# Hengle/AkariRender-1

Hardware: AMD Instinct MI355X
Metric: Msamples/sec (whole node), 10M-tri scene 1080p 1024spp, 1/2/4/8 MI355X (higher is better)
Workload: dtype f32; 1 GPU; C3 synthetic triangle soup (SURVEY.md §8d); triangles=10000002, width=1920, height=1080, spp=1025, max_depth=5, tile=64, parallelism=tile-split x1, bvh_leaf=4, builder=sbvh, form=k_path, ordered_fetch=True

## Files before the change

akarirender-1_amd/csrc/kernels.hip:

```cpp
#include "akr_device.h"
#include "akr_math.h"
#include "kernels.h"

namespace akr {

__device__ __forceinline__ uint32_t fbits(float f) { return __float_as_uint(f); }
__device__ __forceinline__ float bitsf(uint32_t u) { return __uint_as_float(u); }

template <bool TIGHT, bool FAST = false>
__device__ __forceinline__ float box_test(float lox, float hix, float loy, float hiy, float loz, float hiz, V3 o,
                                          V3 invd, float tmin, float tmax) {
    float t0x = (lox - o.x) * invd.x, t1x = (hix - o.x) * invd.x;
    float t0y = (loy - o.y) * invd.y, t1y = (hiy - o.y) * invd.y;
    float t0z = (loz - o.z) * invd.z, t1z = (hiz - o.z) * invd.z;
    float m0, m1, t;
    if (FAST) {
        m0 = fmaxf(fmaxf(fminf(t0x, t1x), fminf(t0y, t1y)), fminf(t0z, t1z));
        m1 = fminf(fminf(fmaxf(t0x, t1x), fmaxf(t0y, t1y)), fmaxf(t0z, t1z));
        t = fmaxf(tmin, m0);
    } else {
        m0 = rmax(rmax(rmin(t0x, t1x), rmin(t0y, t1y)), rmin(t0z, t1z));
        m1 = rmin(rmin(rmax(t0x, t1x), rmax(t0y, t1y)), rmax(t0z, t1z));
        t = rmax(tmin, m0);
    }
// ... 76 lines not shown
    pos_b = bb + lane_prefix(mb);
}

__device__ __forceinline__ void issue_together(const float4 &a, const float4 &b, const float4 &c, const float4 &d,
                                               const float4 &e, const float4 &f) {
    asm volatile("" ::"v"(a.x), "v"(a.y), "v"(a.z), "v"(a.w), "v"(b.x), "v"(b.y), "v"(b.z), "v"(c.x), "v"(c.y),
                 "v"(c.z), "v"(d.x), "v"(d.y), "v"(d.z), "v"(d.w), "v"(e.x), "v"(e.y), "v"(e.z), "v"(f.x), "v"(f.y),
                 "v"(f.z));
}

#define AKR_CHILD_POP 0xFFFFFFFEu
__device__ __forceinline__ bool is_internal(uint32_t c) { return !(c & AKR_CHILD_LEAF); }
__device__ __forceinline__ bool is_leaf(uint32_t c) { return (c & AKR_CHILD_LEAF) && c < AKR_CHILD_POP; }

typedef __attribute__((address_space(3))) unsigned long long lds_u64;
typedef __attribute__((address_space(1))) unsigned long long glb_u64;

constexpr int kStackLdsU64 = kStackLds * kTraceBlock;
__device__ __forceinline__ unsigned long long lds_get(const lds_u64 *s, int e, uint32_t tid) {
    return s[e * kTraceBlock + tid];
}
__device__ __forceinline__ void lds_put(lds_u64 *s, int e, uint32_t tid, unsigned long long v) {
    s[e * kTraceBlock + tid] = v;
}

__device__ __forceinline__ uint32_t stack_pop(const lds_u64 *s_stack, const glb_u64 *ovf, uint32_t ovf_threads,
                                              uint32_t tid, uint32_t gtid, int &sp, float lim) {
    if (__ballot(sp > kStackLds) == 0) {
        while (sp > 0) {
            --sp;
            const unsigned long long e = lds_get(s_stack, sp, tid);
            if (!(__uint_as_float((uint32_t)(e >> 32)) > lim)) return (uint32_t)e;
        }
        return AKR_CHILD_EMPTY;
    }
    while (sp > 0) {
        --sp;
        unsigned long long e;
        if (sp < kStackLds) e = lds_get(s_stack, sp, tid);
        else e = ovf[(size_t)(sp - kStackLds) * ovf_threads + gtid];
        if (!(__uint_as_float((uint32_t)(e >> 32)) > lim)) return (uint32_t)e;
    }
    return AKR_CHILD_EMPTY;
}

template <bool TIGHT, bool FAST, bool ANY>
__device__ __forceinline__ void visit_node(const float4 *nodesf, const uint4 *nodesu, uint32_t &cur, V3 o, V3 d,
                                           V3 invd, float tmin, float tmax, float best, lds_u64 *s_stack, glb_u64 *ovf,
                                           uint32_t ovf_threads, uint32_t tid, uint32_t gtid, int &sp) {
    const float4 q0 = nodesf[4 * (size_t)cur + 0];
    const float4 q1 = nodesf[4 * (size_t)cur + 1];
    const float4 q2 = nodesf[4 * (size_t)cur + 2];
    const uint4 q3 = nodesu[4 * (size_t)cur + 3];
    const float t0 = box_test<TIGHT, FAST>(q0.x, q0.y, q0.z, q0.w, q2.x, q2.y, o, invd, tmin, tmax);
    const float t1 = box_test<TIGHT, FAST>(q1.x, q1.y, q1.z, q1.w, q2.z, q2.w, o, invd, tmin, tmax);
    const float lim = ANY ? tmax : best;
    const bool p0 = !(t0 < 0.0f || t0 > lim);
    const bool p1 = !(t1 < 0.0f || t1 > lim);
    const float dax = q3.z == 0 ? d.x : (q3.z == 1 ? d.y : d.z);
    const bool left_first = dax > 0;
    const uint32_t near_ref = left_first ? q3.x : q3.y;
    const uint32_t far_ref = left_first ? q3.y : q3.x;
    const bool pn = left_first ? p0 : p1;
    const bool pf = left_first ? p1 : p0;
    const float tf = left_first ? t1 : t0;
    if (pn && pf) {
        const unsigned long long e = (unsigned long long)far_ref | ((unsigned long long)__float_as_uint(tf) << 32);
        if (sp < kStackLds) lds_put(s_stack, sp, tid, e);
        else ovf[(size_t)(sp - kStackLds) * ovf_threads + gtid] = e;
        sp++;
    }
    cur = pn ? near_ref : (pf ? far_ref : stack_pop(s_stack, ovf, ovf_threads, tid, gtid, sp, lim));
}

__device__ __forceinline__ float ubyte(uint32_t w, int k) {
    return (float)((w >> (8 * k)) & 0xFFu);
}

template <bool ANY, bool NOPOP = false, bool FIT = false>
__device__ __forceinline__ bool wide_order_push(uint32_t order_lo, uint32_t order_hi, uint32_t dpos, const float (&t)[4],
                                                const bool (&hit)[4], const uint32_t (&ref)[4], uint32_t &cur, float lim,
                                                lds_u64 *s_stack, glb_u64 *ovf, uint32_t ovf_threads, uint32_t tid,
                                                uint32_t gtid, int &sp, lds_u64 *dead = nullptr,
                                                uint32_t *info = nullptr) {
    const uint32_t perm = ((dpos & 4u) ? order_hi : order_lo) >> ((dpos & 3u) << 3);
    const uint32_t pos[4] = {perm & 3u, (perm >> 2) & 3u, (perm >> 4) & 3u, (perm >> 6) & 3u};
    uint32_t pm = 0;
#pragma unroll
    for (int k = 0; k < 4; k++) pm |= hit[k] ? (1u << pos[k]) : 0u;
    if (pm == 0) {
        if constexpr (NOPOP) return true;
        cur = stack_pop(s_stack, ovf, ovf_threads, tid, gtid, sp, lim);
        return false;
    }
    const uint32_t rest = pm & (pm - 1u);
    if (info)
        *info = 1u | (sp + 4 > kStackLds ? 2u : 0u) | (sp + (int)__popc(rest) > kStackLds ? 4u : 0u);
    const bool all_lds = FIT ? __ballot(sp + (int)__popc(rest) > kStackLds) == 0 : __ballot(sp + 4 > kStackLds) == 0;
    if (all_lds) {
#pragma unroll
        for (int k = 0; k < 4; k++) {
            const bool push = (rest >> pos[k]) & 1u;
            const unsigned long long v = (unsigned long long)ref[k] | ((unsigned long long)__float_as_uint(t[k]) << 32);
            if constexpr (FIT) {
                lds_u64 *p = push ? s_stack + (sp + (int)__popc(rest >> (pos[k] + 1u))) * kTraceBlock + tid : dead;
                *p = v;
            } else {
                const int e = sp + (push ? (int)__popc(rest >> (pos[k] + 1u)) : 3);
                lds_put(s_stack, e, tid, v);
            }
        }
    } else {
#pragma unroll
        for (int k = 0; k < 4; k++) {
            if ((rest >> pos[k]) & 1u) {
                const int e = sp + (int)__popc(rest >> (pos[k] + 1u));
                const unsigned long long v = (unsigned long long)ref[k] | ((unsigned long long)__float_as_uint(t[k]) << 32);
                if (e < kStackLds) lds_put(s_stack, e, tid, v);
                else ovf[(size_t)(e - kStackLds) * ovf_threads + gtid] = v;
            }
        }
    }
    sp += (int)__popc(rest);
    const uint32_t first = pm ^ rest;
    uint32_t c = AKR_CHILD_EMPTY;
#pragma unroll
    for (int k = 0; k < 4; k++) c = ((first >> pos[k]) & 1u) ? ref[k] : c;
    cur = c;
    return false;
}

template <bool TIGHT, bool ANY>
__device__ __forceinline__ int visit_wide(const float4 *wn, uint32_t &cur, V3 o, uint32_t dpos, V3 invd, float tmin, float tmax,
                                          float best, lds_u64 *s_stack, glb_u64 *ovf, uint32_t ovf_threads,
                                          uint32_t tid, uint32_t gtid, int &sp) {
    const char *wb = reinterpret_cast<const char *>(wn);
    const uint32_t off = cur << 6;
    const float4 h = *reinterpret_cast<const float4 *>(wb + off);
    const uint4 c = *reinterpret_cast<const uint4 *>(wb + off + 16);
    const uint4 qa = *reinterpret_cast<const uint4 *>(wb + off + 32);
    const uint4 qb = *reinterpret_cast<const uint4 *>(wb + off + 48);
    const uint32_t meta = __float_as_uint(h.w);
    const float sx = __uint_as_float((meta & 0xFFu) << 23);
    const float sy = __uint_as_float(((meta >> 8) & 0xFFu) << 23);
    const float sz = __uint_as_float(((meta >> 16) & 0xFFu) << 23);
    const float lim = ANY ? tmax : best;
    float t[4];
    bool hit[4];
    uint32_t ref[4] = {c.x, c.y, c.z, c.w};
#pragma unroll
    for (int k = 0; k < 4; k++) {
        const float lox = __builtin_fmaf(ubyte(qa.x, k), sx, h.x), hix = __builtin_fmaf(ubyte(qa.y, k), sx, h.x);
        const float loy = __builtin_fmaf(ubyte(qa.z, k), sy, h.y), hiy = __builtin_fmaf(ubyte(qa.w, k), sy, h.y);
        const float loz = __builtin_fmaf(ubyte(qb.x, k), sz, h.z), hiz = __builtin_fmaf(ubyte(qb.y, k), sz, h.z);
        t[k] = box_test<TIGHT, true>(lox, hix, loy, hiy, loz, hiz, o, invd, tmin, tmax);
        hit[k] = ref[k] != AKR_CHILD_EMPTY && !(t[k] < 0.0f || t[k] > lim);
    }
    const int tested = (c.x != AKR_CHILD_EMPTY) + (c.y != AKR_CHILD_EMPTY) + (c.z != AKR_CHILD_EMPTY) +
                       (c.w != AKR_CHILD_EMPTY);
    wide_order_push<ANY>(qb.z, qb.w, dpos, t, hit, ref, cur, lim, s_stack, ovf, ovf_threads, tid, gtid, sp);
    return tested;
}

struct WideNode {
    float4 h;
    uint4 c, qa, qb;
};
__device__ __forceinline__ WideNode wide_load(const float4 *wn, uint32_t cur) {
    const char *wb = reinterpret_cast<const char *>(wn);
    const uint32_t off = cur << 6;
    WideNode nd;
    nd.h = *reinterpret_cast<const float4 *>(wb + off);
    nd.c = *reinterpret_cast<const uint4 *>(wb + off + 16);
    nd.qa = *reinterpret_cast<const uint4 *>(wb + off + 32);
    nd.qb = *reinterpret_cast<const uint4 *>(wb + off + 48);
    return nd;
}

template <bool ANY, bool NOPOP = false, bool FIT = false>
__device__ __forceinline__ int visit_wide_lean_node(const WideNode &nd, uint32_t &cur, V3 o, uint32_t dpos, V3 invd,
                                                    float tmin, float tmaxp, float best, lds_u64 *s_stack, glb_u64 *ovf,
                                                    uint32_t ovf_threads, uint32_t tid, uint32_t gtid, int &sp,
                                                    bool *need_pop = nullptr, lds_u64 *dead = nullptr,
                                                    uint32_t *push_info = nullptr) {
    const float4 h = nd.h;
    const uint4 c = nd.c, qa = nd.qa, qb = nd.qb;
    const uint32_t meta = __float_as_uint(h.w);
    constexpr float kRel = 0x1p-21f;
    constexpr float kAbs = 0x1p-120f;
    const float scx = __uint_as_float((meta & 0xFFu) << 23) * invd.x;
    const float scy = __uint_as_float(((meta >> 8) & 0xFFu) << 23) * invd.y;
    const float scz = __uint_as_float(((meta >> 16) & 0xFFu) << 23) * invd.z;
    const float oqx = (h.x - o.x) * invd.x, oqy = (h.y - o.y) * invd.y, oqz = (h.z - o.z) * invd.z;
    const float ex = __builtin_fmaf(__builtin_fmaf(255.0f, fabsf(scx), fabsf(oqx)), kRel, kAbs);
    const float ey = __builtin_fmaf(__builtin_fmaf(255.0f, fabsf(scy), fabsf(oqy)), kRel, kAbs);
    const float ez = __builtin_fmaf(__builtin_fmaf(255.0f, fabsf(scz), fabsf(oqz)), kRel, kAbs);
    const float nox = oqx - ex, noy = oqy - ey, noz = oqz - ez;
    const float fox = oqx + ex, foy = oqy + ey, foz = oqz + ez;
    const bool px = invd.x > 0.0f, py = invd.y > 0.0f, pz = invd.z > 0.0f;
    const uint32_t qnx = px ? qa.x : qa.y, qfx = px ? qa.y : qa.x;
    const uint32_t qny = py ? qa.z : qa.w, qfy = py ? qa.w : qa.z;
    const uint32_t qnz = pz ? qb.x : qb.y, qfz = pz ? qb.y : qb.x;
    const float lim = ANY ? tmaxp : fminf(best, tmaxp);
    float t[4];
    bool hit[4];
    uint32_t ref[4] = {c.x, c.y, c.z, c.w};
#pragma unroll
    for (int k = 0; k < 4; k++) {
        const float nx = __builtin_fmaf(ubyte(qnx, k), scx, nox), fx = __builtin_fmaf(ubyte(qfx, k), scx, fox);
        const float ny = __builtin_fmaf(ubyte(qny, k), scy, noy), fy = __builtin_fmaf(ubyte(qfy, k), scy, foy);
        const float nz = __builtin_fmaf(ubyte(qnz, k), scz, noz), fz = __builtin_fmaf(ubyte(qfz, k), scz, foz);
        const float tk = fmaxf(fmaxf(nx, ny), fmaxf(nz, tmin));
        const float m1 = fminf(fminf(fx, fy), fminf(fz, lim));
        t[k] = tk;
        hit[k] = ref[k] != AKR_CHILD_EMPTY && tk <= m1;
    }
    const int tested = (c.x != AKR_CHILD_EMPTY) + (c.y != AKR_CHILD_EMPTY) + (c.z != AKR_CHILD_EMPTY) +
                       (c.w != AKR_CHILD_EMPTY);
    const bool np = wide_order_push<ANY, NOPOP, FIT>(qb.z, qb.w, dpos, t, hit, ref, cur, ANY ? tmaxp : best, s_stack, ovf,
                                                     ovf_threads, tid, gtid, sp, dead, push_info);
    if (NOPOP) *need_pop = np;
    return tested;
}

template <bool ANY>
__device__ __forceinline__ int visit_wide_lean(const float4 *wn, uint32_t &cur, V3 o, uint32_t dpos, V3 invd, float tmin,
                                               float tmaxp, float best, lds_u64 *s_stack, glb_u64 *ovf,
                                               uint32_t ovf_threads, uint32_t tid, uint32_t gtid, int &sp) {
    const WideNode nd = wide_load(wn, cur);
    return visit_wide_lean_node<ANY>(nd, cur, o, dpos, invd, tmin, tmaxp, best, s_stack, ovf, ovf_threads, tid, gtid, sp);
}

__device__ __forceinline__ float float_below(float x) {
    const uint32_t b = __float_as_uint(x);
    if (x > 0.0f) return __uint_as_float(b - 1u);
    if (x == 0.0f) return -0x1p-149f;
    return __uint_as_float(b + 1u);
}

__device__ __forceinline__ bool lean_ok(V3 o, V3 invd, float tmin, float tmax) {
    const float mo = fmaxf(fmaxf(fabsf(o.x), fabsf(o.y)), fabsf(o.z));
    const float mi = fmaxf(fmaxf(fabsf(invd.x), fabsf(invd.y)), fabsf(invd.z));
    return fast_box_ok(o, invd, tmin, tmax) && tmin >= 0.0f && tmax > -INFINITY && mo <= 0x1p60f && mi <= 0x1p64f;
}

template <int MODE>
__device__ __forceinline__ void emit_result(const TraceArgs &a, uint32_t idx, float best, float bu, float bv,
                                            uint32_t bgid, bool occluded) {
    constexpr bool ANY = MODE != TRACE_CLOSEST;
    if (MODE == TRACE_SHADOW) {
        if (!occluded) {
            const float4 c = a.shadow_color[idx];
            const uint32_t slot = fbits(c.w);
            float4 l = a.L[slot];
            l.x += c.x;
            l.y += c.y;
            l.z += c.z;
            a.L[slot] = l;
        }
    } else if (a.abi_hits) {
        akr_hit h;
        const bool hit = ANY ? occluded : (bgid != kNoHit);
        h.t = hit ? best : kInf;
        h.u = hit ? bu : 0.0f;
        h.v = hit ? bv : 0.0f;
        h.geom_id = -1;
        h.prim_id = -1;
        if (hit) {
            int lo = 0, hi = a.n_meshes;
            while (hi - lo > 1) {
                const int mid = (lo + hi) / 2;
                if (a.mesh_base[mid] <= bgid) lo = mid; else hi = mid;
            }
            h.geom_id = lo;
            h.prim_id = (int32_t)(bgid - a.mesh_base[lo]);
        }
        h._pad[0] = h._pad[1] = h._pad[2] = 0;
        a.abi_hits[idx] = h;
    } else {
        a.hits[idx] = make_float4(best, bu, bv, bitsf(bgid));
    }
}

template <bool ANY, bool TIGHT>
__device__ __forceinline__ void trace_exact_core(const TraceArgs &a, V3 o, V3 d, V3 invd, float tmin, float tmax,
                                                 lds_u64 *s_stack, glb_u64 *ovf, uint32_t tid, uint32_t gtid, float &best,
                                                 float &bu, float &bv, uint32_t &bgid, bool &occluded) {
    const float4 *nodesf = reinterpret_cast<const float4 *>(a.nodes);
    const uint4 *nodesu = reinterpret_cast<const uint4 *>(a.nodes);
    const float4 r0 = nodesf[0], r2 = nodesf[2];
    const uint32_t root = nodesu[3].x;
    best = kInf;
    bu = bv = 0.0f;
    bgid = kNoHit;
    occluded = false;
    int sp = 0;
    const float tr = box_test<TIGHT, false>(r0.x, r0.y, r0.z, r0.w, r2.x, r2.y, o, invd, tmin, tmax);
    uint32_t cur = (root == AKR_CHILD_EMPTY || tr < 0.0f || tr > (ANY ? tmax : best)) ? AKR_CHILD_EMPTY : root;
    while (cur != AKR_CHILD_EMPTY) {
        if (is_internal(cur)) {
            visit_node<TIGHT, false, ANY>(nodesf, nodesu, cur, o, d, invd, tmin, tmax, best, s_stack, ovf, a.ovf_threads,
                                          tid, gtid, sp);
            continue;
// ... 921 lines not shown
__global__ __launch_bounds__(kBlock) void k_splat_mis(SplatMisArgs m) {
    const SplatArgs &a = m.s;
    const uint32_t i = blockIdx.x * kBlock + threadIdx.x;
    if (i >= a.n) return;
    const uint32_t sl = a.order ? a.order[i] : a.slot_base + i;
    float4 f = a.film[sl];
    float4 l = a.L[sl];
    const float4 e = m.E[sl];
    l.x += e.x;
    l.y += e.y;
    l.z += e.z;
    splat_one(f, l, a.ray_clamp);
    a.film[sl] = f;
}

#ifndef AKR_PATH_WAVES
#define AKR_PATH_WAVES 4
#endif

struct PathRay {
    V3 o, d, invd;
    float tmin, tmax, tmaxp, best, bu, bv;
    uint32_t dpos, bgid, cur, leaf;
    int sp;
};
struct PathCount {
    unsigned long long rays[2] = {0, 0}, box[2] = {0, 0}, tri[2] = {0, 0}, visit[2] = {0, 0}, deep[2] = {0, 0},
                       leaf[2] = {0, 0};
    unsigned long long strav = 0, sleaf = 0, stri = 0, iters = 0;
    unsigned long long tv_issue = 0, tv_wait = 0, tv_comp = 0, tl_issue = 0, tl_wait = 0, tl_comp = 0;
    unsigned long long lphases = 0, lholders = 0;
    unsigned long long pop_iters = 0, pop_rounds = 0, push_iters = 0, push_slow = 0, push_would_fit = 0;
    unsigned long long pop_lane_rounds = 0, pop_lanes = 0;
    bool deep_now = false;
    uint32_t *lines = nullptr;
    uint32_t span[3] = {0, 0, 0};
    const float4 *leaf_base = nullptr;
};

__device__ __forceinline__ void mark_lines(uint32_t *map, uint32_t lo, uint32_t hi, const void *region, const void *p,
                                           uint32_t bytes) {
    const uint64_t r0 = (uint64_t)region >> 7, a = (uint64_t)p;
    if (a < (uint64_t)region) return;
    for (uint64_t l = (a >> 7) - r0; l <= ((a + bytes - 1) >> 7) - r0; l++) {
        const uint64_t b = lo + l;
        if (b < hi) atomicOr(map + (b >> 5), 1u << (b & 31u));
    }
}

template <bool COUNT, bool OVF>
__device__ __forceinline__ void pop_bounded(bool need_pop, PathRay &r, const lds_u64 *s_stack, const glb_u64 *ovf,
                                            uint32_t ovf_threads, uint32_t tid, uint32_t gtid, uint32_t keep,
                                            uint32_t max_rounds, PathCount &c) {
    bool unserved = need_pop;
    uint32_t got = AKR_CHILD_POP;
    int sp = r.sp;
    uint32_t rounds = 0;
    while (true) {
        const bool has = unserved & (sp > 0);
        unsigned long long e;
        if constexpr (!OVF) {
            e = lds_get(s_stack, min(max(sp, 1), kStackLds) - 1, tid);
        } else {
            e = 0;
            if (has) {
                if (sp - 1 < kStackLds) e = lds_get(s_stack, sp - 1, tid);
                else e = ovf[(size_t)(sp - 1 - kStackLds) * ovf_threads + gtid];
            }
        }
        const bool ok = !(__uint_as_float((uint32_t)(e >> 32)) > r.best);
        const uint32_t got_entry = ok ? (uint32_t)e : got, got_none = unserved ? AKR_CHILD_EMPTY : got;
        got = has ? got_entry : got_none;
        sp -= has ? 1 : 0;
        if (COUNT) c.pop_lane_rounds += has ? 1 : 0;
        unserved = has & !ok;
        rounds++;
        if ((uint32_t)__popcll(__ballot(unserved)) < keep || rounds >= max_rounds) break;
    }
    if (COUNT) c.pop_rounds += rounds;
    r.sp = sp;
    if (need_pop) r.cur = got;
}

template <bool COUNT, int EXIT = kWhileExit, bool BOUND = false>
__device__ __forceinline__ void path_traverse(bool busy, int kind, PathRay &r, const float4 *wn, lds_u64 *s_stack,
                                              glb_u64 *ovf, uint32_t ovf_threads, uint32_t tid, uint32_t gtid,
                                              PathCount &c, uint32_t pop_keep = 1, uint32_t pop_rounds = 255,
                                              lds_u64 *dead = nullptr) {
    constexpr bool FIT = BOUND;
    while (true) {
        [[maybe_unused]] unsigned long long tc = 0;
        bool need_pop = false;
        if constexpr (COUNT) {
            c.strav++;
            c.sleaf += busy ? 1 : 0;
            c.iters++;
            const bool vis = busy && is_internal(r.cur);
            const unsigned long long ta = wall_clock64();
            const WideNode nd = wide_load(wn, vis ? r.cur : 0u);
            const unsigned long long tb = wall_clock64();
            asm volatile("s_waitcnt vmcnt(0)" ::: "memory");
            tc = wall_clock64();
            c.tv_issue += tb - ta;
            c.tv_wait += tc - tb;
            uint32_t pinfo = 0;
            if (vis) {
                const uint32_t node = r.cur;
                const int nt = visit_wide_lean_node<false, true, FIT>(nd, r.cur, r.o, r.dpos, r.invd, r.tmin, r.tmaxp,
                                                                      r.best, s_stack, ovf, ovf_threads, tid, gtid, r.sp,
                                                                      &need_pop, dead, &pinfo);
                c.box[kind] += nt;
                c.visit[kind]++;
                c.deep_now = c.deep_now || r.sp > kStackLds;
                if (c.lines)
                    mark_lines(c.lines, 0u, c.span[1], wn, reinterpret_cast<const char *>(wn) + ((size_t)node << 6), 64u);
            }
            if (__ballot(pinfo & 1u) != 0) {
                c.push_iters++;
                if (__ballot(pinfo & 2u) != 0) {
                    c.push_slow++;
                    c.push_would_fit += __ballot(pinfo & 4u) == 0 ? 1 : 0;
                }
            }
        } else if (busy && is_internal(r.cur)) {
            const WideNode nd = wide_load(wn, r.cur);
            visit_wide_lean_node<false, true, FIT>(nd, r.cur, r.o, r.dpos, r.invd, r.tmin, r.tmaxp, r.best, s_stack, ovf,
                                                   ovf_threads, tid, gtid, r.sp, &need_pop, dead);
        }
        if (busy && !need_pop && r.leaf == AKR_CHILD_EMPTY && is_leaf(r.cur)) {
            r.leaf = r.cur;
            need_pop = true;
        }
        if constexpr (BOUND) {
            need_pop = need_pop || (busy && r.cur == AKR_CHILD_POP);
            const unsigned long long want = __ballot(need_pop);
            if (want != 0) {
                if (COUNT) {
                    c.pop_iters++;
                    c.pop_lanes += need_pop ? 1 : 0;
                }
                if (__builtin_expect(__ballot(need_pop && r.sp > kStackLds) == 0, 1))
                    pop_bounded<COUNT, false>(need_pop, r, s_stack, ovf, ovf_threads, tid, gtid, pop_keep, pop_rounds, c);
                else
                    pop_bounded<COUNT, true>(need_pop, r, s_stack, ovf, ovf_threads, tid, gtid, pop_keep, pop_rounds, c);
            }
        } else {
            if (need_pop) r.cur = stack_pop(s_stack, ovf, ovf_threads, tid, gtid, r.sp, r.best);
        }
        const unsigned long long searching = __ballot(busy && r.leaf == AKR_CHILD_EMPTY && r.cur != AKR_CHILD_EMPTY);
        if constexpr (COUNT) {
            const bool stop = (uint32_t)__popcll(searching) <= (uint32_t)EXIT &&
                              (searching == 0 || __ballot(busy && r.leaf != AKR_CHILD_EMPTY) != 0);
            c.tv_comp += wall_clock64() - tc;
            if (stop) break;
        } else if ((uint32_t)__popcll(searching) <= (uint32_t)EXIT &&
                   (searching == 0 || __ballot(busy && r.leaf != AKR_CHILD_EMPTY) != 0)) {
            break;
        }
    }
}

template <bool COUNT>
__device__ __forceinline__ bool leaf_tests(int kind, PathRay &r, const float4 *lr, float4 l0, float4 l1, float4 pa0,
                                           float4 pb0, float4 pc0, float4 pa1, float4 pb1, float4 pc1, PathCount &c) {
    bool hit_any = false;
    const float tl = box_test<true, true>(l0.x, l0.w, l0.y, l1.x, l0.z, l1.y, r.o, r.invd, r.tmin, r.tmax);
// ... 220 lines not shown
        atomicAdd(&q.tv_wait, c.tv_wait);
        atomicAdd(&q.tv_comp, c.tv_comp);
        atomicAdd(&q.tl_issue, c.tl_issue);
        atomicAdd(&q.tl_wait, c.tl_wait);
        atomicAdd(&q.tl_comp, c.tl_comp);
        atomicAdd(&q.leaf_phases, c.lphases);
        atomicAdd(&q.leaf_holders, c.lholders);
        atomicAdd(&q.pop_iters, c.pop_iters);
        atomicAdd(&q.pop_rounds, c.pop_rounds);
        atomicAdd(&q.push_iters, c.push_iters);
        atomicAdd(&q.push_slow, c.push_slow);
        atomicAdd(&q.push_would_fit, c.push_would_fit);
    }
    const unsigned long long plr = wave_sum(c.pop_lane_rounds), pln = wave_sum(c.pop_lanes);
    if (__lane_id() == 0 && pa.prof) {
        atomicAdd(&pa.prof->pop_lane_rounds, plr);
        atomicAdd(&pa.prof->pop_lanes, pln);
    }
    const int slot_of[2] = {TRACE_CLOSEST, TRACE_SHADOW};
    for (int m = 0; m < 2; m++) {
        const unsigned long long rr = wave_sum(c.rays[m]), b = wave_sum(c.box[m]), t = wave_sum(c.tri[m]),
                                 v = wave_sum(c.visit[m]), dp = wave_sum(c.deep[m]), lf = wave_sum(c.leaf[m]);
        if (__lane_id() == 0) {
            TraceCounters &tc = a.counters[slot_of[m]];
            atomicAdd(&tc.rays, rr);
            atomicAdd(&tc.box, b);
            atomicAdd(&tc.tri, t);
            atomicAdd(&tc.visits, v);
            atomicAdd(&tc.deep, dp);
            atomicAdd(&tc.leaves, lf);
        }
    }
    const unsigned long long st = wave_sum(c.strav), sl = wave_sum(c.sleaf), sr = wave_sum(c.stri);
    if (__lane_id() == 0) {
        atomicAdd(&a.counters[TRACE_CLOSEST].slots_trav, st);
        atomicAdd(&a.counters[TRACE_CLOSEST].slots_leaf, sl);
        atomicAdd(&a.counters[TRACE_CLOSEST].slots_tri, sr);
    }
}

template <bool COUNT>
__device__ __forceinline__ uint32_t probe_flags(const PathArgs &pa) {
    if (!COUNT) return AKR_PROBE_SEED;
    uint32_t f = AKR_PROBE_SEED | AKR_PROBE_RAYS;
    if (pa.probe_clock) f |= 4u | (uint32_t)((wall_clock64() >> 4) << 8);
    return f;
}

constexpr int kParkSlots = 8;

template <bool COUNT, bool TAB>
__global__ __launch_bounds__(kTraceBlock) __attribute__((amdgpu_waves_per_eu(AKR_PATH_WAVES))) void k_path(PathArgs pa) {
    if (pa.gate && *pa.gate != pa.gate_want) return;
    const TraceArgs &a = pa.t;
    __shared__ unsigned long long s_stack_mem[kStackLdsU64];
    __shared__ uint32_t s_park[kParkSlots][kTraceBlock];
    __shared__ uint4 s_tab[TAB ? kTabBytes / 16 : 1];
    lds_u64 *s_stack = (lds_u64 *)s_stack_mem;
    glb_u64 *stack_ovf = (glb_u64 *)a.stack_ovf;
    const uint32_t tid = threadIdx.x;
    const uint32_t gtid = blockIdx.x * kTraceBlock + tid;
    const uint32_t n = pa.n_pix;
    const int nb = pa.max_depth == 0 ? 1 : pa.max_depth;
    const bool ff = a.any_far_first != 0;
    const auto tab = PathTab<TAB>::make(pa.sc, s_tab);
    static_assert(kParkSlots >= 1 && kTraceBlock % 64 == 0, "the push's scratch words lie in a wave's park row 0");
    lds_u64 *dead = (lds_u64 *)&s_park[0][0] + (tid >> 1);
    PathCount c;
    if (COUNT) {
        c.lines = pa.lines;
        c.span[1] = pa.lines_span[1];
        c.span[2] = pa.lines_span[2];
        c.leaf_base = a.wide_leaves;
    }
    PixelFetch f{blockIdx.x % kWorkShards, 0, 0, (int)kWorkShards, n == 0};
    f.s_lo = shard_begin(n, f.shard);
    f.s_hi = shard_begin(n, f.shard + 1);

    uint32_t pix = 0, left = 0, seed = 0, pxr = 0;
    int depth = 0;
    V3 beta{1.0f, 1.0f, 1.0f}, Lr{0.0f, 0.0f, 0.0f}, scol{0.0f, 0.0f, 0.0f};
    float4 film = {0.0f, 0.0f, 0.0f, 0.0f};
    float4 pe0 = {}, pe1 = {};
    bool pend = false;
    bool any = false;
    bool need_pixel = true, done = false, fin = false, busy = false;
    uint32_t pc_closest = 0, pc_shadow = 0;
    PathRay r{};
    r.best = kInf;
    r.bgid = kNoHit;
    r.cur = r.leaf = AKR_CHILD_EMPTY;
    unsigned long long p_outer = 0, p_procs = 0, p_tp = 0, p_tt = 0, p_tl = 0, p_lanes = 0, p_t0 = 0, p_t = 0, p_tsh = 0;
    unsigned long long p_tpark = 0, p_tnext = 0, p_tbegin = 0, p_tload = 0;
    if (COUNT) p_t0 = wall_clock64();

    while (true) {
        const unsigned long long waiting = __ballot(!busy && !done);
        const uint32_t nwait = (uint32_t)__popcll(waiting);
        const uint32_t nbusy = (uint32_t)__popcll(__ballot(busy));
        if (nwait == 0 && nbusy == 0) break;
        if (COUNT) {
            p_outer++;
            p_t = wall_clock64();
        }
        if (nwait > 0 && 64u * nwait >= pa.min_wait * (nwait + nbusy)) {
            if (COUNT) {
                p_procs++;
                p_lanes += nwait;
            }
            path_park(s_park, tid, r);
            __builtin_amdgcn_fence(__ATOMIC_RELEASE, "workgroup");
            asm volatile("" ::: "memory");
            bool fresh = false, next_any = false, sample_end = false, start = false;
            float4 ra = {}, rb = {};
            unsigned long long p_ts = 0;
            unsigned long long tl_phase = 0;
            if (COUNT) {
                p_ts = wall_clock64();
                p_tpark += p_ts - p_t;
            }
            if (!busy && !done && fin) {
                fin = false;
                const uint32_t hgid = r.bgid;
                if (any) {
                    if (hgid == kNoHit) {
                        Lr.x += scol.x;
                        Lr.y += scol.y;
                        Lr.z += scol.z;
                    }
                    if (pend) {
                        ra = pe0;
                        rb = pe1;
                        fresh = true;
                        pend = false;
                    } else {
                        sample_end = true;
                    }
                } else if (hgid == kNoHit) {
                    sample_end = true;
                } else {
                    const V3 wo{-bitsf(s_park[3][tid]), -bitsf(s_park[4][tid]), -bitsf(s_park[5][tid])};
                    Bounce bo;
                    if (COUNT && pa.lines)
                        mark_lines(pa.lines, pa.lines_span[2], pa.lines_span[3], pa.sc.tri, pa.sc.tri + hgid,
                                   (uint32_t)sizeof(ShadeTri));
                    shade_hit_tab(pa.sc, tab, hgid, r.bu, r.bv, wo, beta, seed, depth,
                              pa.max_depth, depth == nb - 1, bo, COUNT ? &tl_phase : nullptr);
                    if (bo.emit) {
                        Lr.x += bo.e.x;
                        Lr.y += bo.e.y;
                        Lr.z += bo.e.z;
                    }
                    if (bo.ext) {
                        beta = bo.nb;
                        depth++;
                    }
                    if (bo.sh) {
                        ra = bo.s0;
                        rb = bo.s1;
                        scol = bo.col;
                        next_any = true;
                        fresh = true;
                        pend = bo.ext;
                        pe0 = bo.e0;
                        pe1 = bo.e1;
                    } else if (bo.ext) {
                        ra = bo.e0;
                        rb = bo.e1;
                        fresh = true;
                    } else {
                        sample_end = true;
                    }
                }
            }
            if (COUNT) {
                const unsigned long long t = wall_clock64();
                p_tsh += t - p_ts;
                p_ts = t;
                p_tload += wave_max(tl_phase);
            }
            if (sample_end) {
                splat_one(film, make_float4(Lr.x, Lr.y, Lr.z, 0.0f), pa.ray_clamp);
                if (--left == 0) {
                    pa.film[pix] = film;
                    if (pa.state_out) pa.state_out[pix] = seed;
                    if (pa.probe)
                        pa.probe[pix] = make_uint4(seed, COUNT ? pc_closest : 0u, COUNT ? pc_shadow : 0u,
                                                   probe_flags<COUNT>(pa));
                    need_pixel = true;
                } else {
                    start = true;
                }
            }
            const bool asked = need_pixel && !done;
            fetch_pixels(f, n, pa.work, pa.order ? pa.order_mode : FETCH_LINEAR, pa.order, pa.prio, need_pixel, done, pix);
            if (asked && !need_pixel) {
                const uint32_t px = pa.pixel[pix];
                pxr = px;
                left = pa.spp;
                if (pa.state_in) {
                    seed = pa.state_in[pix];
                    film = pa.film[pix];
                } else {
                    seed = (uint32_t)((int)(px & 0xFFFFu) + (int)(px >> 16) * pa.cam.width);
                    film = make_float4(0.0f, 0.0f, 0.0f, 0.0f);
                }
                start = true;
                if (COUNT) pc_closest = pc_shadow = 0;
            }
            if (start) {
                Lr = V3{0.0f, 0.0f, 0.0f};
                beta = V3{1.0f, 1.0f, 1.0f};
                depth = 0;
                const uint32_t px = pxr;
                camera_ray(pa.cam, (int)(px & 0xFFFFu), (int)(px >> 16), seed, ra, rb);
                fresh = true;
            }
            asm volatile("" ::: "memory");
            if (COUNT) {
                const unsigned long long t = wall_clock64();
                p_tnext += t - p_ts;
                p_ts = t;
            }
            path_unpark(s_park, tid, r, ff, any);
            if (fresh) {
                any = next_any;
                if (COUNT) {
                    pc_closest += any ? 0u : 1u;
                    pc_shadow += any ? 1u : 0u;
                }
                busy = path_begin<COUNT>(a, any, ra, rb, r, s_stack, stack_ovf, tid, gtid, c);
                fin = !busy;
            }
            if (COUNT) p_tbegin += wall_clock64() - p_ts;
        }
        if (COUNT) {
            const unsigned long long t = wall_clock64();
            p_tp += t - p_t;
            p_t = t;
        }
        if (!__any(busy)) continue;
        const int kd = any ? 1 : 0;
        path_traverse<COUNT, kWhileExitPath, true>(busy, kd, r, a.wide_nodes, s_stack, stack_ovf, a.ovf_threads, tid, gtid,
                                                   c, pa.pop_keep, pa.pop_rounds, dead);
        if (COUNT) {
            const unsigned long long t = wall_clock64();
            p_tt += t - p_t;
            p_t = t;
        }
        const bool hit_any = path_leaf<COUNT>(busy, kd, r, a.wide_leaves, c);
        if (busy && (hit_any || r.cur == AKR_CHILD_EMPTY)) {
            busy = false;
            fin = true;
            if (COUNT) c.deep[kd] += c.deep_now ? 1 : 0;
        }
        if (COUNT) p_tl += wall_clock64() - p_t;
    }
    if (COUNT) {
        path_count_flush(pa, c, p_outer, p_procs, p_tp, p_tt, p_tl, p_t0, p_lanes, p_tsh);
        if (__lane_id() == 0 && pa.prof) {
            atomicAdd(&pa.prof->tp_park, p_tpark);
            atomicAdd(&pa.prof->tp_next, p_tnext);
            atomicAdd(&pa.prof->tp_begin, p_tbegin);
            atomicAdd(&pa.prof->tp_load, p_tload);
        }
    }
}

__device__ __forceinline__ void path_park(uint32_t (*s_park)[kTraceBlock], uint32_t tid, const PathRay &r) {
    const float pv[8] = {r.o.x, r.o.y, r.o.z, r.d.x, r.d.y, r.d.z, r.tmin, r.tmax};
#pragma unroll
    for (int k = 0; k < 8; k++) s_park[k][tid] = fbits(pv[k]);
}
__device__ __forceinline__ void path_unpark(uint32_t (*s_park)[kTraceBlock], uint32_t tid, PathRay &r, bool far_first,
                                            bool occl) {
    r.o = V3{bitsf(s_park[0][tid]), bitsf(s_park[1][tid]), bitsf(s_park[2][tid])};
    r.d = V3{bitsf(s_park[3][tid]), bitsf(s_park[4][tid]), bitsf(s_park[5][tid])};
    r.tmin = bitsf(s_park[6][tid]);
    r.tmax = bitsf(s_park[7][tid]);
    r.invd = V3{1.0f / r.d.x, 1.0f / r.d.y, 1.0f / r.d.z};
    r.dpos = (r.d.x > 0.0f ? 1u : 0u) | (r.d.y > 0.0f ? 2u : 0u) | (r.d.z > 0.0f ? 4u : 0u);
    if (occl && far_first) r.dpos ^= 7u;
    r.tmaxp = float_below(r.tmax);
    r.leaf = AKR_CHILD_EMPTY;
}

__device__ __forceinline__ int nth_set_bit(unsigned long long m, uint32_t r) {
    int base = 0;
#pragma unroll
    for (int s = 32; s > 0; s >>= 1) {
        const unsigned long long low = m & ((1ull << s) - 1ull);
        const uint32_t c = (uint32_t)__popcll(low);
        if (r >= c) {
            r -= c;
            m >>= s;
            base += s;
        } else {
            m = low;
        }
    }
    return base;
}

constexpr uint32_t kDeferSlots = 8;
enum : uint32_t { RAY_NONE = 0, RAY_OWN = 1, RAY_OWN_SHADOW = 2, RAY_FOREIGN = 3 };

struct DeferState {
    uint32_t w = 0;
    static constexpr uint32_t KIND = 0, RP = 2, LAST = 3, OPEN = 4, NSH = 6, DEPTH = 14, FTAG = 18, PEND = 30, RUN = 31;
    __device__ __forceinline__ uint32_t get(uint32_t off, uint32_t bits) const { return (w >> off) & ((1u << bits) - 1u); }
    __device__ __forceinline__ void set(uint32_t off, uint32_t bits, uint32_t v) {
        const uint32_t m = ((1u << bits) - 1u) << off;
        w = (w & ~m) | ((v << off) & m);
    }
    __device__ __forceinline__ uint32_t kind() const { return get(KIND, 2); }
    __device__ __forceinline__ uint32_t rp() const { return get(RP, 1); }
    __device__ __forceinline__ uint32_t last() const { return get(LAST, 1); }
    __device__ __forceinline__ uint32_t open() const { return get(OPEN, 2); }
    __device__ __forceinline__ uint32_t nsh(uint32_t q) const { return get(NSH + 4 * q, 4); }
    __device__ __forceinline__ int depth() const { return (int)get(DEPTH, 4); }
    __device__ __forceinline__ uint32_t ftag() const { return get(FTAG, 12); }
    __device__ __forceinline__ bool pend() const { return get(PEND, 1) != 0; }
    __device__ __forceinline__ bool running() const { return get(RUN, 1) != 0; }
};

template <bool COUNT, bool TAB>
__global__ __launch_bounds__(kTraceBlock) __attribute__((amdgpu_waves_per_eu(AKR_PATH_WAVES))) void k_path_defer(PathArgs pa) {
    if (pa.gate && *pa.gate != pa.gate_want) return;
    const TraceArgs &a = pa.t;
    __shared__ unsigned long long s_stack_mem[kStackLdsU64];
    __shared__ uint32_t s_park[kParkSlots][kTraceBlock];
    __shared__ uint4 s_tab[TAB ? kTabBytes / 16 : 1];
    __shared__ uint32_t s_res[kTraceBlock];
    lds_u64 *s_stack = (lds_u64 *)s_stack_mem;
    glb_u64 *stack_ovf = (glb_u64 *)a.stack_ovf;
    const uint32_t tid = threadIdx.x;
    const uint32_t gtid = blockIdx.x * kTraceBlock + tid;
    const size_t lanes = (size_t)gridDim.x * kTraceBlock;
// ... 1168 lines not shown
```

Before: 531.9 Msamples/s.

## Add wave-mask traversal loop and pack path state flags into one register

```diff
diff --git a/akarirender-1_amd/csrc/kernels.hip b/akarirender-1_amd/csrc/kernels.hip
--- a/akarirender-1_amd/csrc/kernels.hip
+++ b/akarirender-1_amd/csrc/kernels.hip
@@ -182,12 +182,13 @@
                                                 const bool (&hit)[4], const uint32_t (&ref)[4], uint32_t &cur, float lim,
                                                 lds_u64 *s_stack, glb_u64 *ovf, uint32_t ovf_threads, uint32_t tid,
                                                 uint32_t gtid, int &sp, lds_u64 *dead = nullptr,
-                                                uint32_t *info = nullptr) {
+                                                uint32_t *info = nullptr, uint32_t *entered = nullptr) {
     const uint32_t perm = ((dpos & 4u) ? order_hi : order_lo) >> ((dpos & 3u) << 3);
     const uint32_t pos[4] = {perm & 3u, (perm >> 2) & 3u, (perm >> 4) & 3u, (perm >> 6) & 3u};
     uint32_t pm = 0;
 #pragma unroll
     for (int k = 0; k < 4; k++) pm |= hit[k] ? (1u << pos[k]) : 0u;
+    if (entered) *entered = pm;
     if (pm == 0) {
         if constexpr (NOPOP) return true;
         cur = stack_pop(s_stack, ovf, ovf_threads, tid, gtid, sp, lim);
@@ -197,7 +198,7 @@
     if (info)
         *info = 1u | (sp + 4 > kStackLds ? 2u : 0u) | (sp + (int)__popc(rest) > kStackLds ? 4u : 0u);
     const bool all_lds = FIT ? __ballot(sp + (int)__popc(rest) > kStackLds) == 0 : __ballot(sp + 4 > kStackLds) == 0;
-    if (all_lds) {
+    if (FIT ? __builtin_expect(all_lds, 1) : all_lds) {
 #pragma unroll
         for (int k = 0; k < 4; k++) {
             const bool push = (rest >> pos[k]) & 1u;
@@ -282,7 +283,7 @@
                                                     float tmin, float tmaxp, float best, lds_u64 *s_stack, glb_u64 *ovf,
                                                     uint32_t ovf_threads, uint32_t tid, uint32_t gtid, int &sp,
                                                     bool *need_pop = nullptr, lds_u64 *dead = nullptr,
-                                                    uint32_t *push_info = nullptr) {
+                                                    uint32_t *push_info = nullptr, uint32_t *entered = nullptr) {
     const float4 h = nd.h;
     const uint4 c = nd.c, qa = nd.qa, qb = nd.qb;
     const uint32_t meta = __float_as_uint(h.w);
@@ -318,7 +319,7 @@
     const int tested = (c.x != AKR_CHILD_EMPTY) + (c.y != AKR_CHILD_EMPTY) + (c.z != AKR_CHILD_EMPTY) +
                        (c.w != AKR_CHILD_EMPTY);
     const bool np = wide_order_push<ANY, NOPOP, FIT>(qb.z, qb.w, dpos, t, hit, ref, cur, ANY ? tmaxp : best, s_stack, ovf,
-                                                     ovf_threads, tid, gtid, sp, dead, push_info);
+                                                     ovf_threads, tid, gtid, sp, dead, push_info, entered);
     if (NOPOP) *need_pop = np;
     return tested;
 }
@@ -1406,6 +1407,71 @@
     if (need_pop) r.cur = got;
 }
 
+__device__ __forceinline__ unsigned long long mask_of(bool cmp) { return __builtin_amdgcn_ballot_w64(cmp); }
+__device__ __forceinline__ bool in_mask(unsigned long long m) { return __builtin_amdgcn_inverse_ballot_w64(m); }
+__device__ __forceinline__ uint32_t lane_count(unsigned long long m) {
+    uint32_t n = (uint32_t)__popcll(m);
+    asm("" : "+s"(n));
+    return n;
+}
+
+__device__ __forceinline__ void pop_bounded_lds(unsigned long long need, PathRay &r, const lds_u64 *s_stack, uint32_t tid,
+                                                uint32_t keep, uint32_t max_rounds) {
+    unsigned long long unserved = need;
+    uint32_t got = AKR_CHILD_POP;
+    int sp = r.sp;
+    uint32_t rounds = 0;
+    while (true) {
+        const unsigned long long has = unserved & mask_of(sp > 0);
+        const unsigned long long e = lds_get(s_stack, min(max(sp, 1), kStackLds) - 1, tid);
+        const unsigned long long cull = mask_of(__uint_as_float((uint32_t)(e >> 32)) > r.best);
+        got = in_mask(unserved & ~has) ? AKR_CHILD_EMPTY : got;
+        got = in_mask(has & ~cull) ? (uint32_t)e : got;
+        sp -= in_mask(has) ? 1 : 0;
+        unserved = has & cull;
+        rounds++;
+        if (lane_count(unserved) < (rounds < max_rounds ? keep : 65u)) break;
+    }
+    r.sp = sp;
+    r.cur = in_mask(need) ? got : r.cur;
+}
+
+template <int EXIT>
+__device__ __forceinline__ void path_traverse_masks(unsigned long long bm, PathRay &r, const float4 *wn, lds_u64 *s_stack,
+                                                    glb_u64 *ovf, uint32_t ovf_threads, uint32_t tid, uint32_t gtid,
+                                                    uint32_t pop_keep, uint32_t pop_rounds, lds_u64 *dead) {
+    static_assert(EXIT >= 0 && EXIT < 64, "the exit test below counts a searching lane without a holder as 65");
+    PathCount none;
+    while (true) {
+        uint32_t pm = 1u;
+        [[maybe_unused]] bool np;
+        if (in_mask(bm & mask_of(is_internal(r.cur)))) {
+            const WideNode nd = wide_load(wn, r.cur);
+            visit_wide_lean_node<false, true, true>(nd, r.cur, r.o, r.dpos, r.invd, r.tmin, r.tmaxp, r.best, s_stack, ovf,
+                                                    ovf_threads, tid, gtid, r.sp, &np, dead, nullptr, &pm);
+        }
+        asm("" : "+v"(pm));
+        unsigned long long need = mask_of(pm == 0);
+        const unsigned long long no_leaf = mask_of(r.leaf == AKR_CHILD_EMPTY);
+        const unsigned long long post = bm & ~need & no_leaf & mask_of(is_leaf(r.cur));
+        r.leaf = in_mask(post) ? r.cur : r.leaf;
+        need |= post | (bm & mask_of(r.cur == AKR_CHILD_POP));
+        if (need != 0) {
+            if (__builtin_expect((need & mask_of(r.sp > kStackLds)) == 0, 1))
+                pop_bounded_lds(need, r, s_stack, tid, pop_keep, pop_rounds);
+            else
+                pop_bounded<false, true>(in_mask(need), r, s_stack, ovf, ovf_threads, tid, gtid, pop_keep, pop_rounds, none);
+        }
+        const unsigned long long free_now = bm & no_leaf & ~post;
+        const unsigned long long searching = free_now & mask_of(r.cur != AKR_CHILD_EMPTY);
+        const unsigned long long holders = bm & ~free_now;
+        const uint32_t n = lane_count(searching);
+        uint32_t left = holders != 0 ? n : n * 65u;
+        asm("" : "+s"(left));
+        if (left <= (uint32_t)EXIT) break;
+    }
+}
+
 template <bool COUNT, int EXIT = kWhileExit, bool BOUND = false>
 __device__ __forceinline__ void path_traverse(bool busy, int kind, PathRay &r, const float4 *wn, lds_u64 *s_stack,
                                               glb_u64 *ovf, uint32_t ovf_threads, uint32_t tid, uint32_t gtid,
@@ -1792,9 +1858,8 @@
     V3 beta{1.0f, 1.0f, 1.0f}, Lr{0.0f, 0.0f, 0.0f}, scol{0.0f, 0.0f, 0.0f};
     float4 film = {0.0f, 0.0f, 0.0f, 0.0f};
     float4 pe0 = {}, pe1 = {};
-    bool pend = false;
-    bool any = false;
-    bool need_pixel = true, done = false, fin = false, busy = false;
+    enum : uint32_t { F_BUSY = 1u, F_DONE = 2u, F_FIN = 4u, F_NEED = 8u, F_ANY = 16u, F_PEND = 32u };
+    uint32_t fl = F_NEED;
     uint32_t pc_closest = 0, pc_shadow = 0;
     PathRay r{};
     r.best = kInf;
@@ -1805,9 +1870,9 @@
     if (COUNT) p_t0 = wall_clock64();
 
     while (true) {
-        const unsigned long long waiting = __ballot(!busy && !done);
+        const unsigned long long waiting = mask_of((fl & (F_BUSY | F_DONE)) == 0);
         const uint32_t nwait = (uint32_t)__popcll(waiting);
-        const uint32_t nbusy = (uint32_t)__popcll(__ballot(busy));
+        const uint32_t nbusy = (uint32_t)__popcll(mask_of((fl & F_BUSY) != 0));
         if (nwait == 0 && nbusy == 0) break;
         if (COUNT) {
             p_outer++;
@@ -1818,6 +1883,8 @@
                 p_procs++;
                 p_lanes += nwait;
             }
+            bool busy = (fl & F_BUSY) != 0, done = (fl & F_DONE) != 0, fin = (fl & F_FIN) != 0;
+            bool need_pixel = (fl & F_NEED) != 0, any = (fl & F_ANY) != 0, pend = (fl & F_PEND) != 0;
             path_park(s_park, tid, r);
             __builtin_amdgcn_fence(__ATOMIC_RELEASE, "workgroup");
             asm volatile("" ::: "memory");
@@ -1942,6 +2009,9 @@
                 busy = path_begin<COUNT>(a, any, ra, rb, r, s_stack, stack_ovf, tid, gtid, c);
                 fin = !busy;
             }
+            fl = (busy ? F_BUSY : 0u) | (done ? F_DONE : 0u) | (fin ? F_FIN : 0u) | (need_pixel ? F_NEED : 0u) |
+                 (any ? F_ANY : 0u) | (pend ? F_PEND : 0u);
+            asm("" : "+v"(fl));
             if (COUNT) p_tbegin += wall_clock64() - p_ts;
         }
         if (COUNT) {
@@ -1949,21 +2019,25 @@
             p_tp += t - p_t;
             p_t = t;
         }
-        if (!__any(busy)) continue;
-        const int kd = any ? 1 : 0;
-        path_traverse<COUNT, kWhileExitPath, true>(busy, kd, r, a.wide_nodes, s_stack, stack_ovf, a.ovf_threads, tid, gtid,
-                                                   c, pa.pop_keep, pa.pop_rounds, dead);
+        const unsigned long long bm = mask_of((fl & F_BUSY) != 0);
+        if (bm == 0) continue;
+        const bool busy = in_mask(bm);
+        const int kd = (fl & F_ANY) != 0 ? 1 : 0;
+        if constexpr (COUNT)
+            path_traverse<COUNT, kWhileExitPath, true>(busy, kd, r, a.wide_nodes, s_stack, stack_ovf, a.ovf_threads, tid,
+                                                       gtid, c, pa.pop_keep, pa.pop_rounds, dead);
+        else
+            path_traverse_masks<kWhileExitPath>(bm, r, a.wide_nodes, s_stack, stack_ovf, a.ovf_threads, tid, gtid,
+                                                pa.pop_keep, pa.pop_rounds, dead);
         if (COUNT) {
             const unsigned long long t = wall_clock64();
             p_tt += t - p_t;
             p_t = t;
         }
         const bool hit_any = path_leaf<COUNT>(busy, kd, r, a.wide_leaves, c);
-        if (busy && (hit_any || r.cur == AKR_CHILD_EMPTY)) {
-            busy = false;
-            fin = true;
-            if (COUNT) c.deep[kd] += c.deep_now ? 1 : 0;
-        }
+        const bool ended = busy && (hit_any || r.cur == AKR_CHILD_EMPTY);
+        fl = ended ? (fl ^ (F_BUSY | F_FIN)) : fl;
+        if (COUNT && ended) c.deep[kd] += c.deep_now ? 1 : 0;
         if (COUNT) p_tl += wall_clock64() - p_t;
     }
     if (COUNT) {
```

After: 571.7 Msamples/s, median of 6. +7.5%, better.
